# MoseleyBioinformaticsLab/pdb_eda

Measured on NVIDIA B200. Metric: voxels/s (atom-sphere voxels + blob-CCL voxels per pass of the voxel hot path), higher is better.
Workload: dtype f64

## Files before the change

include/pdbeda_b200.h:

```cpp
#ifndef PDBEDA_B200_H
#define PDBEDA_B200_H

#include <stdint.h>

#ifdef __cplusplus
extern "C" {
#endif

#define PE_ABI_VERSION 1

typedef enum pe_status {
    PE_OK = 0,
    PE_ERR_ARG = -1,
    PE_ERR_CUDA = -2,
    PE_ERR_CAPACITY = -3,
    PE_ERR_NO_DEVICE = -4
} pe_status;

typedef struct pe_geom {
    int32_t ncrs[3];
    int32_t crs_start[3];
    int32_t xyz_interval[3];
    int32_t crs_interval[3];
    int32_t unique_ncrs[3];
    int32_t map2xyz[3];
    int32_t map2crs[3];
    int32_t orthogonal;
    int32_t mv_perm[3];
    int32_t mv_fma;
    double grid_length[3];
    double origin[3];
    double ortho[9];
    double deortho[9];
} pe_geom;

int pe_abi_version(void);
const char *pe_last_error(void);
int pe_device_info(int32_t *sm_count, int32_t *cc_major, int32_t *cc_minor);

long long pe_launch_count(void);
void pe_profile_enable(int on);
void pe_profile_reset(void);
int pe_profile_entries(void);
int pe_profile_get(int index, const char **name, long long *count, double *total_ms);

int64_t pe_stats_workspace_bytes(void);
int pe_map_mean_std(const float *d_rho, int64_t n, double *d_out, void *d_ws, void *stream);
int pe_map_sum_abs(const float *d_rho, int64_t n, float cutoff, double *d_out, void *d_ws, void *stream);
int pe_sum_abs_f64(const double *d_values, int64_t n, float cutoff, double *d_out, void *d_ws, void *stream);

int pe_point_density(const pe_geom *g, const float *d_rho, int64_t n, const int32_t *d_crs, float *d_rho_out,
                     uint8_t *d_valid, void *stream);
int pe_xyz2crs(const pe_geom *g, int64_t n, const double *d_xyz, int32_t *d_crs, void *stream);
int pe_crs2xyz(const pe_geom *g, int64_t n, const int32_t *d_crs, double *d_xyz, void *stream);

#define PE_SPHERE_NOUT 8
int64_t pe_sphere_workspace_bytes(int64_t n_atoms);
int pe_sphere_union_warp_cycles(unsigned long long *out5);
int pe_sphere_sums(const pe_geom *g, const float *d_rho, int32_t n_atoms, const double *d_xyz,
                   const float *d_radius, int32_t n_groups, const int32_t *d_group_start, float cut_pos,
                   float cut_neg, double *d_out, void *d_ws, void *stream);
int pe_sphere_sums_atoms_and_groups(const pe_geom *g, const float *d_rho, int32_t n_atoms, const double *d_xyz,
                                    const float *d_atom_radius, float max_atom_radius, const float *d_group_radius,
                                    int32_t n_groups, const int32_t *d_group_start, float cut_pos, float cut_neg,
                                    double *d_out_atoms, double *d_out_groups, void *d_ws, void *stream);

typedef struct pe_sums_map {
    pe_geom geom;
    const float *d_rho;
    float cut_pos;
    float cut_neg;
} pe_sums_map;
int64_t pe_batch_sphere_sums_workspace_bytes(int64_t n_atoms);
int pe_batch_sphere_sums(int32_t n_maps, const pe_sums_map *d_maps, int32_t n_atoms, const double *d_xyz, const float *d_radius,
                         int32_t n_groups, const int32_t *d_group_map, const int32_t *d_group_start, const int32_t *d_atom_start,
                         double *d_out, void *d_ws, void *stream);

int pe_sphere_count(const pe_geom *g, const float *d_rho, int32_t n_atoms, const double *d_xyz,
                    const float *d_radius, float cutoff, int32_t *d_count, int32_t *d_box, void *stream);
int pe_sphere_fill(const pe_geom *g, const float *d_rho, int32_t n_atoms, const double *d_xyz,
                   const float *d_radius, float cutoff, const int64_t *d_offset, int32_t max_box_voxels,
                   int32_t *d_index, float *d_value, int32_t *d_label, void *stream);

int64_t pe_blob_workspace_bytes(const pe_geom *g, int64_t cap_voxels);
int pe_blob_stage_times(unsigned long long *out12);
int pe_blob_label(const pe_geom *g, const float *d_rho, float cut_pos, float cut_neg, int64_t cap_voxels,
                  int64_t cap_blobs, int64_t *d_counts, uint32_t *d_key, float *d_value, int32_t *d_label,
                  double *d_stats, void *d_ws, void *stream);

int64_t pe_slab_exchange_bytes(int64_t cap_blobs, int64_t cap_plane);
int64_t pe_slab_workspace_bytes(int32_t world, int64_t cap_blobs, int32_t u0, int32_t u1);
int pe_slab_boundary(const pe_geom *g_slab, int32_t u2_whole, int32_t s0, int32_t last_is_cut, const int64_t *d_counts,
                     int64_t cap_voxels, const uint32_t *d_key, const int32_t *d_label, int64_t cap_blobs, int64_t cap_plane,
                     void *d_exchange, void *d_ws, void *stream);
int pe_slab_merge(int32_t world, int32_t rank, const void *d_gathered, int64_t cap_blobs, int64_t cap_plane, int32_t u0,
                  int32_t u1, int32_t *d_new_number, int64_t *d_n_merged, void *d_ws, void *stream);
int pe_slab_relabel(const pe_geom *g_whole, int32_t u2_slab, int32_t s0, const int64_t *d_counts, int64_t cap_voxels,
                    const uint32_t *d_key, const float *d_value, int32_t *d_label, int64_t cap_blobs,
                    const int32_t *d_new_number, const int64_t *d_n_merged, int64_t cap_merged, double *d_stats, void *d_ws,
                    void *stream);
int pe_slab_status(const void *d_ws, void *stream, int32_t *bad);

int64_t pe_cluster_workspace_bytes(int64_t n);
int pe_cluster_crs(int64_t n, const int32_t *d_crs, int32_t *d_label, int64_t *d_nclusters, void *d_ws,
                   void *stream);
int pe_cluster_crs_grouped(int64_t n, const int32_t *d_crs, const int32_t *d_group, int32_t *d_label,
                           uint8_t *d_first, int64_t *d_nclusters, void *d_ws, void *stream);

int pe_crs_stats(const pe_geom *g, const float *d_rho, int64_t n, const int32_t *d_crs, const int32_t *d_label,
                 const uint8_t *d_take, int64_t n_clusters, double *d_stats, void *stream);

int pe_pair_metrics(const pe_geom *g, const float *d_rho_fo, const float *d_rho_diff, int64_t n, const int32_t *d_crs,
                    const int32_t *d_label, const uint8_t *d_take, int64_t n_groups, double *d_out, void *stream);

typedef struct pe_pair_map {
    pe_geom geom;
    const float *d_fo;
    const float *d_diff;
} pe_pair_map;
int64_t pe_pair_union_workspace_bytes(int32_t n_atoms);
int pe_pair_union_metrics(int32_t n_maps, const pe_pair_map *d_maps, int32_t n_groups, const int32_t *d_group_map,
                          const int32_t *d_group_start, const double *d_xyz, const float *d_radius, double *d_out, void *d_ws,
                          void *stream);

int64_t pe_overlap_workspace_bytes(int64_t n, int64_t cap_pairs);
int pe_overlap_pairs(int64_t n, const int32_t *d_crs, const int32_t *d_owner, const int32_t *d_group,
                     int64_t cap_pairs, int64_t *d_npairs, int32_t *d_pairs, void *d_ws, void *stream);

typedef struct pe_batch_map {
    pe_geom geom;
    const float *d_rho;
    float cutoff;
    int32_t atom_begin, atom_end;
    int32_t reserved;
} pe_batch_map;
int64_t pe_cloud_workspace_bytes(int64_t n_atoms, int64_t n_entries, int64_t n_residues, int64_t n_maps);
int pe_cloud_count(int32_t n_maps, const pe_batch_map *d_maps, int32_t n_atoms, const int32_t *d_atom_map, const double *d_xyz,
                   const float *d_radius, uint32_t *d_offset, int64_t *d_totals, void *d_scan_ws, uint32_t *d_box_bits, void *stream);
int pe_cloud_aggregate(int32_t n_maps, const pe_batch_map *d_maps, int32_t n_atoms, const int32_t *d_atom_map,
                       const double *d_xyz, const float *d_radius, const int32_t *d_atom_residue,
                       const int32_t *d_atom_local, const uint64_t *d_atom_bonded, const double *d_atom_electrons,
                       int32_t n_residues, const uint32_t *d_offset, int64_t n_entries, int32_t max_box_voxels,
                       double min_cloud_electrons, const uint32_t *d_box_bits, double *d_atom_out, double *d_map_out, void *d_ws,
                       void *stream);
int pe_cloud_status(const void *d_ws, void *stream, int32_t *bad);
int pe_cloud_statistics(int32_t n_maps, const pe_batch_map *d_maps, int32_t n_atoms, const double *d_atom_out,
                        const double *d_map_out, const double *d_atom_static, const int32_t *d_perm, int32_t n_segments,
                        const int32_t *d_seg_map, const int32_t *d_seg_type, const int32_t *d_seg_begin,
                        const int32_t *d_seg_end, int32_t max_segment, const double *d_unit_volume,
                        const double *d_current_slopes, double min_total_electrons, double *d_scratch, double *d_seg_out,
                        double *d_map_stats, void *stream);

int64_t pe_symmetry_workspace_bytes(int32_t n_atoms, int32_t n_ops);
int pe_symmetry_expand(const pe_geom *g, int32_t n_atoms, const double *d_xyz, int32_t n_ops, const double *d_rot,
                       const double *d_shift, const double *lo, const double *hi, int64_t cap, int64_t *d_count,
                       int32_t *d_atom, int32_t *d_image, double *d_out_xyz, void *d_ws, void *stream);

int pe_nearest_atom(int64_t n_blobs, const double *d_centroid, int64_t n_atoms, const double *d_coords,
                    int32_t *d_idx, double *d_dist, void *stream);

#ifdef __cplusplus
}
#endif
#endif
```

pdb_eda_b200/_lib.py:

```python
import ctypes
import os

_HERE = os.path.dirname(os.path.abspath(__file__))
LIB_PATH = os.path.join(_HERE, "csrc", "libpdbeda_b200.so")

PE_SPHERE_NOUT = 8


class PeGeom(ctypes.Structure):
    _fields_ = [
        ("ncrs", ctypes.c_int32 * 3),
        ("crs_start", ctypes.c_int32 * 3),
        ("xyz_interval", ctypes.c_int32 * 3),
        ("crs_interval", ctypes.c_int32 * 3),
        ("unique_ncrs", ctypes.c_int32 * 3),
        ("map2xyz", ctypes.c_int32 * 3),
        ("map2crs", ctypes.c_int32 * 3),
        ("orthogonal", ctypes.c_int32),
        ("mv_perm", ctypes.c_int32 * 3),
        ("mv_fma", ctypes.c_int32),
        ("grid_length", ctypes.c_double * 3),
        ("origin", ctypes.c_double * 3),
        ("ortho", ctypes.c_double * 9),
        ("deortho", ctypes.c_double * 9),
    ]


class PeBatchMap(ctypes.Structure):
    _fields_ = [("geom", PeGeom), ("d_rho", ctypes.c_void_p), ("cutoff", ctypes.c_float), ("atom_begin", ctypes.c_int32),
                ("atom_end", ctypes.c_int32), ("reserved", ctypes.c_int32)]


class PeSumsMap(ctypes.Structure):
    _fields_ = [("geom", PeGeom), ("d_rho", ctypes.c_void_p), ("cut_pos", ctypes.c_float), ("cut_neg", ctypes.c_float)]


class PePairMap(ctypes.Structure):
    _fields_ = [("geom", PeGeom), ("d_fo", ctypes.c_void_p), ("d_diff", ctypes.c_void_p)]


class PdbEdaLibError(RuntimeError):
    pass


_P = ctypes.c_void_p
_I32 = ctypes.c_int32
_I64 = ctypes.c_int64
_F32 = ctypes.c_float
_GEOM = ctypes.POINTER(PeGeom)

SIGNATURES = {
    "pe_abi_version": (ctypes.c_int, []),
    "pe_last_error": (ctypes.c_char_p, []),
    "pe_device_info": (ctypes.c_int, [ctypes.POINTER(_I32)] * 3),
    "pe_launch_count": (ctypes.c_longlong, []),
    "pe_profile_enable": (None, [ctypes.c_int]),
    "pe_profile_reset": (None, []),
    "pe_profile_entries": (ctypes.c_int, []),
    "pe_profile_get": (ctypes.c_int, [ctypes.c_int, ctypes.POINTER(ctypes.c_char_p), ctypes.POINTER(ctypes.c_longlong),
                                      ctypes.POINTER(ctypes.c_double)]),
    "pe_stats_workspace_bytes": (_I64, []),
    "pe_map_mean_std": (ctypes.c_int, [_P, _I64, _P, _P, _P]),
    "pe_map_sum_abs": (ctypes.c_int, [_P, _I64, _F32, _P, _P, _P]),
    "pe_sum_abs_f64": (ctypes.c_int, [_P, _I64, _F32, _P, _P, _P]),
    "pe_point_density": (ctypes.c_int, [_GEOM, _P, _I64, _P, _P, _P, _P]),
    "pe_xyz2crs": (ctypes.c_int, [_GEOM, _I64, _P, _P, _P]),
    "pe_crs2xyz": (ctypes.c_int, [_GEOM, _I64, _P, _P, _P]),
    "pe_sphere_workspace_bytes": (_I64, [_I64]),
    "pe_sphere_union_warp_cycles": (ctypes.c_int, [ctypes.POINTER(ctypes.c_ulonglong)]),
    "pe_sphere_sums": (ctypes.c_int, [_GEOM, _P, _I32, _P, _P, _I32, _P, _F32, _F32, _P, _P, _P]),
    "pe_sphere_sums_atoms_and_groups": (ctypes.c_int, [_GEOM, _P, _I32, _P, _P, _F32, _P, _I32, _P, _F32, _F32, _P, _P, _P, _P]),
    "pe_sphere_count": (ctypes.c_int, [_GEOM, _P, _I32, _P, _P, _F32, _P, _P, _P]),
    "pe_sphere_fill": (ctypes.c_int, [_GEOM, _P, _I32, _P, _P, _F32, _P, _I32, _P, _P, _P, _P]),
    "pe_blob_workspace_bytes": (_I64, [_GEOM, _I64]),
    "pe_blob_stage_times": (ctypes.c_int, [ctypes.POINTER(ctypes.c_ulonglong)]),
    "pe_blob_label": (ctypes.c_int, [_GEOM, _P, _F32, _F32, _I64, _I64, _P, _P, _P, _P, _P, _P, _P]),
    "pe_cluster_workspace_bytes": (_I64, [_I64]),
    "pe_cluster_crs": (ctypes.c_int, [_I64, _P, _P, _P, _P, _P]),
    "pe_cluster_crs_grouped": (ctypes.c_int, [_I64, _P, _P, _P, _P, _P, _P, _P]),
    "pe_crs_stats": (ctypes.c_int, [_GEOM, _P, _I64, _P, _P, _P, _I64, _P, _P]),
    "pe_pair_metrics": (ctypes.c_int, [_GEOM, _P, _P, _I64, _P, _P, _P, _I64, _P, _P]),
    "pe_batch_sphere_sums_workspace_bytes": (_I64, [_I64]),
    "pe_batch_sphere_sums": (ctypes.c_int, [_I32, _P, _I32, _P, _P, _I32, _P, _P, _P, _P, _P, _P]),
    "pe_pair_union_workspace_bytes": (_I64, [_I32]),
    "pe_pair_union_metrics": (ctypes.c_int, [_I32, _P, _I32, _P, _P, _P, _P, _P, _P, _P]),
    "pe_overlap_workspace_bytes": (_I64, [_I64, _I64]),
    "pe_overlap_pairs": (ctypes.c_int, [_I64, _P, _P, _P, _I64, _P, _P, _P, _P]),
    "pe_symmetry_workspace_bytes": (_I64, [_I32, _I32]),
    "pe_symmetry_expand": (ctypes.c_int, [_GEOM, _I32, _P, _I32, _P, _P, ctypes.POINTER(ctypes.c_double),
                                          ctypes.POINTER(ctypes.c_double), _I64, _P, _P, _P, _P, _P, _P]),
    "pe_nearest_atom": (ctypes.c_int, [_I64, _P, _I64, _P, _P, _P, _P]),
    "pe_slab_exchange_bytes": (_I64, [_I64, _I64]),
    "pe_slab_workspace_bytes": (_I64, [_I32, _I64, _I32, _I32]),
    "pe_slab_boundary": (ctypes.c_int, [_GEOM, _I32, _I32, _I32, _P, _I64, _P, _P, _I64, _I64, _P, _P, _P]),
    "pe_slab_merge": (ctypes.c_int, [_I32, _I32, _P, _I64, _I64, _I32, _I32, _P, _P, _P, _P]),
    "pe_slab_relabel": (ctypes.c_int, [_GEOM, _I32, _I32, _P, _I64, _P, _P, _P, _I64, _P, _P, _I64, _P, _P, _P]),
    "pe_slab_status": (ctypes.c_int, [_P, _P, ctypes.POINTER(_I32)]),
    "pe_cloud_workspace_bytes": (_I64, [_I64, _I64, _I64, _I64]),
    "pe_cloud_count": (ctypes.c_int, [_I32, _P, _I32, _P, _P, _P, _P, _P, _P, _P, _P]),
    "pe_cloud_aggregate": (ctypes.c_int, [_I32, _P, _I32, _P, _P, _P, _P, _P, _P, _P, _I32, _P, _I64, _I32, ctypes.c_double, _P, _P, _P,
                                          _P, _P]),
    "pe_cloud_status": (ctypes.c_int, [_P, _P, ctypes.POINTER(_I32)]),
    "pe_cloud_statistics": (ctypes.c_int, [_I32, _P, _I32, _P, _P, _P, _P, _I32, _P, _P, _P, _P, _I32, _P, _P, ctypes.c_double, _P, _P,
                                           _P, _P]),
}

_lib = None


def load():
    global _lib
    if _lib is not None:
        return _lib
    if not os.path.isfile(LIB_PATH):
        raise PdbEdaLibError(
            "%s not found: build it with `python -c 'import __graft_entry__ as g; g.build()'` or "
            "`make -C pdb_eda_b200/csrc` (there is no CPU fallback)" % LIB_PATH)
    lib = ctypes.CDLL(LIB_PATH)
    for name, (restype, argtypes) in SIGNATURES.items():
        fn = getattr(lib, name)
        fn.restype = restype
        fn.argtypes = argtypes
    if lib.pe_abi_version() != 1:
        raise PdbEdaLibError("libpdbeda_b200.so ABI version %d, expected 1" % lib.pe_abi_version())
    _lib = lib
    return lib


def check(rc, what):
    if rc != 0:
        msg = load().pe_last_error()
        raise PdbEdaLibError("%s failed (%d): %s" % (what, rc, msg.decode("utf-8", "replace") if msg else "?"))


def require_device():
    lib = load()
    sm, major, minor = _I32(0), _I32(0), _I32(0)
    check(lib.pe_device_info(ctypes.byref(sm), ctypes.byref(major), ctypes.byref(minor)), "pe_device_info")
    return sm.value, major.value, minor.value


def profile(enable=None, reset=False):
    lib = load()
    if reset:
        lib.pe_profile_reset()
    if enable is not None:
        lib.pe_profile_enable(1 if enable else 0)
        return None
    out = {}
    for i in range(lib.pe_profile_entries()):
        name, count, ms = ctypes.c_char_p(), ctypes.c_longlong(0), ctypes.c_double(0.0)
        if lib.pe_profile_get(i, ctypes.byref(name), ctypes.byref(count), ctypes.byref(ms)) == 0:
            out[name.value.decode()] = (count.value, ms.value)
    return out


def launch_count():
    return load().pe_launch_count()
```

pdb_eda_b200/csrc/pe_blob.cu:

```cuda
#include <cooperative_groups.h>
#include "pe_common.cuh"

namespace cg = cooperative_groups;

namespace pe {

constexpr int kBmpTx = 32;
constexpr int kBmpTy = 8;
constexpr int kSparseThreads = 512;
constexpr int kSegShift = 9;
constexpr int kSegWords = 1 << kSegShift;
constexpr int kChunkShift = 9;
constexpr int kChunkSmem = 4096;
constexpr int kScanBlocksPerSm = 2;
constexpr int kQueueCap = 160;
constexpr int kPoolWords = (kSparseThreads / 32) * 3 * kQueueCap > kChunkSmem ? (kSparseThreads / 32) * 3 * kQueueCap : kChunkSmem;
static_assert((1 << kChunkShift) == kSparseThreads, "a ranking chunk is one block of voxels");

struct BlobPlan {
    int U0, U1, U2, W;
    int64_t nwords;
    int64_t nwords_pad;
    int64_t nseg;
    int64_t cap;
// ... 88 lines not shown
                }
            }
        } else {
            for (int j = 0; j < nbits; ++j) {
#pragma unroll
                for (int i = 0; i < VEC; ++i) {
                    const float e = (i == 0 || c + i < NC) ? __ldg(p + (int64_t)j * plane + i) : 0.f;
                    pos[i] |= (e >= cpos) ? (1u << j) : 0u;
                    neg[i] |= (e <= cneg) ? (1u << j) : 0u;
                }
            }
        }
#pragma unroll
        for (int i = 0; i < VEC; ++i) {
            accp[i][q] = use_pos ? pos[i] : 0u;
            accn[i][q] = use_neg ? neg[i] : 0u;
        }
    }
#pragma unroll
    for (int i = 0; i < VEC; ++i) {
        if (c + i < U0) {
            const int64_t widx = ((int64_t)(c + i) * U1 + r) * W + w_begin;
            *reinterpret_cast<uint4 *>(bmp_pos + widx) = make_uint4(accp[i][0], accp[i][1], accp[i][2], accp[i][3]);
            *reinterpret_cast<uint4 *>(bmp_neg + widx) = make_uint4(accn[i][0], accn[i][1], accn[i][2], accn[i][3]);
            const int np = __popc(accp[i][0]) + __popc(accp[i][1]) + __popc(accp[i][2]) + __popc(accp[i][3]);
            const int nn = __popc(accn[i][0]) + __popc(accn[i][1]) + __popc(accn[i][2]) + __popc(accn[i][3]);
            if (np) atomicAdd(segcount + (widx >> kSegShift), (uint32_t)np);
            if (nn) atomicAdd(segcount + ((nwords_pad + widx) >> kSegShift), (uint32_t)nn);
        }
    }
}

__device__ unsigned long long g_stage_ns[12];
__device__ __forceinline__ void stamp(int i) {
    if (blockIdx.x == 0 && threadIdx.x == 0) {
        unsigned long long t;
        asm volatile("mov.u64 %0, %%globaltimer;" : "=l"(t));
        g_stage_ns[i] = t;
    }
}

struct SparseArgs {
    const float *rho;
    int NC, NR, U1, U2, W;
    int64_t nwords_pad, cap, cap_blobs;
    int nseg;
    int p1_blocks;
    int p1_per_sm;
    int *sm_rank;
    const uint32_t *bmp;
    const uint32_t *segcount;
    uint32_t *base;
    uint32_t *parent;
    uint2 *flags;
    uint32_t *coarse;
    int64_t nchunk_cap;
    int64_t *counts;
    uint32_t *key;
    float *value;
    int32_t *label;
    double *stats;
};

__device__ __forceinline__ uint32_t block_sum_u32(uint32_t v, uint32_t *smem ) {
    const int lane = threadIdx.x & 31, w = threadIdx.x >> 5;
    v = (uint32_t)warp_sum((int)v);
    __syncthreads();
    if (lane == 0) smem[w] = v;
    __syncthreads();
    uint32_t t = 0;
    for (int i = 0; i < (int)(blockDim.x >> 5); ++i) t += smem[i];
    return t;
}

__device__ __forceinline__ uint32_t uf_union_root(uint32_t *parent, uint32_t a, uint32_t b) {
    for (;;) {
        a = uf_find_halve(parent, a);
        b = uf_find_halve(parent, b);
        if (a == b) return a;
        if (a < b) {
            const uint32_t t = a;
            a = b;
            b = t;
        }
        const uint32_t old = atomicMin(parent + a, b);
        if (old == a) return b;
        a = old;
    }
}

__device__ __forceinline__ uint32_t roots_below(const uint2 *__restrict__ flags, const uint32_t *cpre, uint32_t x) {
    const uint2 f = __ldcg(flags + (x >> 5));
    return cpre[x >> kChunkShift] + f.y + (uint32_t)__popc(f.x & ((1u << (x & 31u)) - 1u));
}

__global__ void __launch_bounds__(kSparseThreads, 3) blob_sparse_kernel(const __grid_constant__ pe_geom g, const SparseArgs a) {
    cg::grid_group grid = cg::this_grid();
    __shared__ uint32_t smem[32];
    __shared__ uint32_t pool[kPoolWords];
    uint32_t *cpre_s = pool;
    const int lane = threadIdx.x & 31, warp = threadIdx.x >> 5;
    const int nb = gridDim.x, b = blockIdx.x;
    const int warps_per_block = kSparseThreads >> 5;
    stamp(0);

    uint32_t n0 = 0, n_all = 0;
    __shared__ int scan_index;
    if (threadIdx.x == 0) {
        unsigned smid;
        asm volatile("mov.u32 %0, %%smid;" : "=r"(smid));
        int idx = -1;
        if (a.p1_blocks >= nb) idx = b;
        else if (atomicAdd(a.sm_rank + (smid < 254u ? smid : 254u), 1) < a.p1_per_sm) idx = atomicAdd(a.sm_rank + 255, 1);
        scan_index = idx;
    }
    __syncthreads();
    const int bi = scan_index;
    if (bi >= 0 && bi < a.p1_blocks) {
        const int nwarps = a.p1_blocks * warps_per_block;
        const int spw = (a.nseg + nwarps - 1) / nwarps;
        const int seg_class1 = (int)(a.nwords_pad >> kSegShift);
        const int sb = min(bi * warps_per_block * spw, a.nseg);
        {
            const int seg_begin = min(sb + warp * spw, a.nseg), seg_end = min(seg_begin + spw, a.nseg);
            for (int64_t i = ((int64_t)seg_begin << kSegShift) + 32 * lane; i < ((int64_t)seg_end << kSegShift); i += 32 * 32)
                asm volatile("prefetch.global.L2 [%0];" ::"l"(a.bmp + i));
        }
        uint32_t before;
        {
            uint32_t s_before = 0, s0 = 0, s_all = 0;
            constexpr int kBatch = 8;
            for (int i0 = threadIdx.x; i0 < a.nseg; i0 += kSparseThreads * kBatch) {
                uint32_t v[kBatch];
#pragma unroll
                for (int j = 0; j < kBatch; ++j) {
                    const int i = i0 + j * kSparseThreads;
                    v[j] = i < a.nseg ? __ldg(a.segcount + i) : 0u;
                }
#pragma unroll
                for (int j = 0; j < kBatch; ++j) {
                    const int i = i0 + j * kSparseThreads;
                    s_all += v[j];
                    if (i < sb) s_before += v[j];
                    if (i < seg_class1) s0 += v[j];
                }
            }
            before = block_sum_u32(s_before, smem);
            n0 = block_sum_u32(s0, smem);
            n_all = block_sum_u32(s_all, smem);
        }
        const bool overflow = (int64_t)n0 > a.cap || (int64_t)(n_all - n0) > a.cap;
        if (bi == 0 && threadIdx.x == 0) {
            a.counts[0] = (int64_t)n0;
            a.counts[2] = (int64_t)(n_all - n0);
            if (overflow) a.counts[4] = 1;
        }
        if (!overflow) {
            const int seg_begin = min(sb + warp * spw, a.nseg), seg_end = min(seg_begin + spw, a.nseg);
            uint32_t mine = 0;
            for (int i = sb + lane; i < seg_begin; i += 32) mine += a.segcount[i];
            uint32_t run = before + (uint32_t)warp_sum((int)mine);
            uint32_t carry = 0u;
            if (seg_begin < seg_end && seg_begin > 0) carry = a.bmp[((int64_t)seg_begin << kSegShift) - 1];
            const int64_t w_end = (int64_t)seg_end << kSegShift;
            uint32_t *queue = pool + warp * (3 * kQueueCap);
            int qn = 0;
            uint4 next = make_uint4(0u, 0u, 0u, 0u);
            if (seg_begin < seg_end) next = __ldcg(reinterpret_cast<const uint4 *>(a.bmp + ((int64_t)seg_begin << kSegShift) + 4 * lane));
            for (int64_t i0 = (int64_t)seg_begin << kSegShift; i0 < w_end; i0 += 128) {
                const int64_t widx0 = i0 + 4 * lane;
                const uint4 wv = next;
                if (i0 + 128 < w_end) next = __ldcg(reinterpret_cast<const uint4 *>(a.bmp + widx0 + 128));
                const int c4 = __popc(wv.x) + __popc(wv.y) + __popc(wv.z) + __popc(wv.w);
                const int excl = warp_excl_scan(c4, lane);
                uint32_t p = run + (uint32_t)excl;
                run += (uint32_t)__shfl_sync(kFull, excl + c4, 31);
                uint32_t prevw = __shfl_up_sync(kFull, wv.w, 1);
                if (lane == 0) prevw = carry;
                carry = __shfl_sync(kFull, wv.w, 31);
                const uint32_t words[4] = {wv.x, wv.y, wv.z, wv.w};
#pragma unroll
                for (int q = 0; q < 4; ++q) {
                    const uint32_t word = words[q];
                    const unsigned act = __ballot_sync(kFull, word != 0u);
                    if (word) {
                        const int slot = qn + __popc(act & ((1u << lane) - 1u));
                        const uint32_t pw = q == 0 ? prevw : words[q > 0 ? q - 1 : 0];
                        queue[slot] = (uint32_t)(widx0 + q);
                        queue[kQueueCap + slot] = p | (pw & 0x80000000u);
                        queue[2 * kQueueCap + slot] = word;
                        p += (uint32_t)__popc(word);
                    }
                    qn += __popc(act);
                }
                const bool last = i0 + 128 >= w_end;
                if (qn <= kQueueCap - 128 && !last) continue;
                __syncwarp();
                for (int e = lane; e < qn; e += 32) {
                    const uint32_t widx = queue[e], pp = queue[kQueueCap + e], word = queue[2 * kQueueCap + e];
                    const uint32_t p_first = pp & 0x7fffffffu;
                    const int k = (int64_t)widx >= a.nwords_pad ? 1 : 0;
                    const uint32_t local = widx - (k ? (uint32_t)a.nwords_pad : 0u);
                    const uint32_t colrow = local / (uint32_t)a.W;
                    const int w = (int)(local - colrow * (uint32_t)a.W);
                    const int64_t out0 = (int64_t)k * a.cap - (k ? (int64_t)n0 : 0);
                    const bool prev_last = (w > 0) && (pp >> 31);
                    a.base[widx] = p_first;
                    const uint32_t starts = word & ~((word << 1) | (prev_last ? 1u : 0u));
                    const uint32_t keybase = colrow * (uint32_t)a.U2 + (uint32_t)w * 32u;
                    uint32_t rest = word, pv = p_first;
                    while (rest) {
                        const int bit = __ffs(rest) - 1;
                        rest &= rest - 1;
                        const uint32_t below = starts & ((2u << bit) - 1u);
                        uint32_t par;
                        if (below) {
                            const int sbit = 31 - __clz(below);
                            par = p_first + (uint32_t)__popc(word & ((1u << sbit) - 1u));
                        } else {
                            par = p_first - 1;
                        }
                        a.key[out0 + pv] = keybase + (uint32_t)bit;
                        a.parent[pv] = par;
                        ++pv;
                    }
                }
                qn = 0;
                __syncwarp();
            }
        }
    }
    grid.sync();
    stamp(1);
    if (!(bi >= 0 && bi < a.p1_blocks)) {
        n0 = (uint32_t)__ldcg(a.counts + 0);
        n_all = n0 + (uint32_t)__ldcg(a.counts + 2);
    }
    if (a.p1_blocks < nb && __ldcg(a.sm_rank + 255) != a.p1_blocks) {
        if (b == 0 && threadIdx.x == 0) a.counts[4] = 2;
        return;
    }
    if (__ldcg(a.counts + 4) != 0) return;
    const int64_t n = (int64_t)n_all;
    const uint32_t n1 = n_all - n0;

    const int64_t gstride = (int64_t)nb * kSparseThreads;
    const int64_t gtid = (int64_t)b * kSparseThreads + threadIdx.x;
    {
        const int64_t rows0 = min((int64_t)n0, a.cap_blobs) * 8, rows1 = min((int64_t)n1, a.cap_blobs) * 8;
        for (int64_t i = gtid; i < rows0; i += gstride) a.stats[i] = 0.0;
        for (int64_t i = gtid; i < rows1; i += gstride) a.stats[a.cap_blobs * 8 + i] = 0.0;
    }
    for (int64_t i = gtid; i < n; i += gstride) {
        const int k = i >= (int64_t)n0 ? 1 : 0;
        const int64_t oi = (int64_t)k * a.cap + (i - (k ? (int64_t)n0 : 0));
        const uint32_t kk = __ldcg(a.key + oi);
        const int s = (int)(kk % (uint32_t)a.U2);
        const uint32_t colrow = kk / (uint32_t)a.U2;
        const int r = (int)(colrow % (uint32_t)a.U1), c = (int)(colrow / (uint32_t)a.U1);
        const int w = s >> 5, bit = s & 31;
        const uint32_t *bmp = a.bmp + (k ? a.nwords_pad : 0);
        const uint32_t *base = a.base + (k ? a.nwords_pad : 0);
        const float dens = __ldg(a.rho + ((int64_t)s * a.NR + r) * a.NC + c);
        int64_t nw[4];
        bool ok[4];
        ok[0] = c > 0 && r > 0;
        ok[1] = c > 0;
        ok[2] = c > 0 && r + 1 < a.U1;
        ok[3] = r > 0;
        nw[0] = ((int64_t)(c - 1) * a.U1 + r - 1) * a.W + w;
        nw[1] = nw[0] + a.W;
        nw[2] = nw[1] + a.W;
        nw[3] = ((int64_t)c * a.U1 + r - 1) * a.W + w;
        uint32_t B[4], Bm[4], Bp[4];
#pragma unroll
        for (int j = 0; j < 4; ++j) {
            B[j] = ok[j] ? __ldcg(bmp + nw[j]) : 0u;
            Bm[j] = (ok[j] && bit == 0 && w > 0) ? __ldcg(bmp + nw[j] - 1) : 0u;
            Bp[j] = (ok[j] && bit == 31 && w + 1 < a.W) ? __ldcg(bmp + nw[j] + 1) : 0u;
        }
        uint32_t sel[4];
#pragma unroll
        for (int j = 0; j < 4; ++j) {
            uint32_t m = 0;
            if ((B[j] >> bit) & 1u) {
                m = 1u;
            } else {
                if (bit > 0 && ((B[j] >> (bit - 1)) & 1u)) m |= 2u;
                if (bit < 31 && ((B[j] >> (bit + 1)) & 1u)) m |= 4u;
                if (Bm[j] >> 31) m |= 8u;
                if (Bp[j] & 1u) m |= 16u;
            }
            sel[j] = m;
        }
        if (sel[1] & 1u) {
            sel[0] = sel[2] = sel[3] = 0u;
        } else if (sel[3] & 1u) {
            sel[0] = sel[1] = 0u;
        } else if (sel[0] & 1u) {
            sel[1] = sel[3] = 0u;
        } else if (sel[2] & 1u) {
            sel[1] = 0u;
        } else {
#pragma unroll
            for (int side = 0; side < 2; ++side) {
                const uint32_t bits = side ? (4u | 16u) : (2u | 8u);
                if (sel[1] & bits) {
                    sel[0] &= ~bits;
// ... 43 lines not shown
        }
        const uint32_t fw = __ballot_sync(kFull, isroot);
        if (lane == 0) wcnt[warp] = (uint32_t)__popc(fw);
        __syncthreads();
        uint32_t fine = 0, tot = 0;
        for (int j = 0; j < warps_per_block; ++j) {
            const uint32_t v = wcnt[j];
            if (j < warp) fine += v;
            tot += v;
        }
        if (lane == 0) a.flags[(chunk << (kChunkShift - 5)) + warp] = make_uint2(fw, fine);
        if (threadIdx.x == 0) a.coarse[chunk] = tot;
        __syncthreads();
    }
    grid.sync();
    stamp(3);

    const uint32_t *cpre = cpre_s;
    uint32_t n_roots;
    if (nchunks <= kChunkSmem) {
        constexpr int kPer = kChunkSmem / kSparseThreads;
        uint32_t v[kPer], sum = 0;
#pragma unroll
        for (int j = 0; j < kPer; ++j) {
            const int64_t ci = (int64_t)threadIdx.x * kPer + j;
            v[j] = ci < nchunks ? __ldcg(a.coarse + ci) : 0u;
            sum += v[j];
        }
        const uint32_t wex = (uint32_t)warp_excl_scan((int)sum, lane);
        __syncthreads();
        if (lane == 31) wcnt[warp] = wex + sum;
        __syncthreads();
        uint32_t off = wex;
        uint32_t all = 0;
        for (int j = 0; j < warps_per_block; ++j) {
            const uint32_t t = wcnt[j];
            if (j < warp) off += t;
            all += t;
        }
#pragma unroll
        for (int j = 0; j < kPer; ++j) {
            cpre_s[threadIdx.x * kPer + j] = off;
            off += v[j];
        }
        n_roots = all;
        __syncthreads();
    } else {
        uint32_t *gpre = a.coarse + a.nchunk_cap;
        if (b == 0) {
            __shared__ uint32_t carry_s;
            if (threadIdx.x == 0) carry_s = 0u;
            __syncthreads();
            for (int64_t c0 = 0; c0 < nchunks; c0 += kSparseThreads) {
                const int64_t ci = c0 + threadIdx.x;
                const uint32_t v = ci < nchunks ? __ldcg(a.coarse + ci) : 0u;
                const uint32_t wex = (uint32_t)warp_excl_scan((int)v, lane);
                if (lane == 31) wcnt[warp] = wex + v;
                __syncthreads();
                uint32_t off = carry_s + wex, all = 0;
                for (int j = 0; j < warps_per_block; ++j) {
                    const uint32_t t = wcnt[j];
                    if (j < warp) off += t;
                    all += t;
                }
                if (ci < nchunks) gpre[ci] = off;
                __syncthreads();
                if (threadIdx.x == 0) carry_s += all;
                __syncthreads();
            }
            if (threadIdx.x == 0) gpre[nchunks] = carry_s;
        }
        grid.sync();
        cpre = gpre;
        n_roots = __ldcg(gpre + nchunks);
    }
    const uint32_t nb0 = n0 == n_all ? n_roots : roots_below(a.flags, cpre, n0);
    const uint32_t nb1 = n_roots - nb0;
    if (b == 0 && threadIdx.x == 0) {
        a.counts[1] = (int64_t)nb0;
        a.counts[3] = (int64_t)nb1;
    }
    if ((int64_t)nb0 > a.cap_blobs || (int64_t)nb1 > a.cap_blobs) {
        if (b == 0 && threadIdx.x == 0) a.counts[4] = 1;
        return;
    }
    for (int64_t i0 = gtid - lane; i0 < n; i0 += gstride) {
        const int64_t i = i0 + lane;
        const bool live = i < n;
        int32_t blob = -1;
        double v[8] = {0, 0, 0, 0, 0, 0, 0, 0};
        if (live) {
            const int k = i >= (int64_t)n0 ? 1 : 0;
            const int64_t oi = (int64_t)k * a.cap + (i - (k ? (int64_t)n0 : 0));
            const uint32_t gr = roots_below(a.flags, cpre, __ldcg(a.parent + i));
            blob = (int32_t)(gr - (k ? nb0 : 0u));
            a.label[oi] = blob;
            blob += k ? (int32_t)a.cap_blobs : 0;
            const uint32_t kk = __ldcg(a.key + oi);
            const int s = (int)(kk % (uint32_t)a.U2);
            const uint32_t colrow = kk / (uint32_t)a.U2;
            const int r = (int)(colrow % (uint32_t)a.U1), c = (int)(colrow / (uint32_t)a.U1);
            double x, y, z;
            crs2xyz(g, c, r, s, x, y, z);
            const double d = (double)__ldcg(a.value + oi);
            v[0] = 1.0;
            v[1] = d;
            v[2] = __dmul_rn(d, x);
            v[3] = __dmul_rn(d, y);
            v[4] = __dmul_rn(d, z);
            v[5] = x;
            v[6] = y;
            v[7] = z;
        }
        const int32_t prev = __shfl_up_sync(kFull, blob, 1);
        const bool head = (lane == 0) || (prev != blob);
        const unsigned heads = __ballot_sync(kFull, head);
        const int segno = __popc(heads & (0xffffffffu >> (31 - lane)));
#pragma unroll
        for (int o = 1; o < 32; o <<= 1) {
            const int seg_o = __shfl_down_sync(kFull, segno, o);
            const bool take = (lane + o < 32) && (seg_o == segno);
#pragma unroll
            for (int q = 0; q < 8; ++q) {
                const double other = __shfl_down_sync(kFull, v[q], o);
                if (take) v[q] += other;
            }
        }
        if (live && head) {
            double *st = a.stats + (int64_t)blob * 8;
#pragma unroll
            for (int q = 0; q < 8; ++q) atomicAdd(st + q, v[q]);
        }
    }
    stamp(4);
}

}

using namespace pe;

extern "C" {

int pe_blob_stage_times(unsigned long long *out12) {
    PE_CHECK_ARG(out12 != nullptr, "pe_blob_stage_times: null pointer");
    PE_CUDA(cudaMemcpyFromSymbol(out12, g_stage_ns, sizeof(unsigned long long) * 12));
    return PE_OK;
}

int64_t pe_blob_workspace_bytes(const pe_geom *g, int64_t cap_voxels) {
    if (!g || cap_voxels < 0) return -1;
    return make_plan(g, cap_voxels).total;
}

int pe_blob_label(const pe_geom *g, const float *d_rho, float cut_pos, float cut_neg, int64_t cap_voxels,
                  int64_t cap_blobs, int64_t *d_counts, uint32_t *d_key, float *d_value, int32_t *d_label,
                  double *d_stats, void *d_ws, void *stream) {
    if (int rc = check_geom(g)) return rc;
    PE_CHECK_ARG(d_rho && d_counts && d_key && d_value && d_label && d_stats && d_ws, "pe_blob_label: null pointer");
    PE_CHECK_ARG(cap_voxels > 0 && cap_blobs > 0, "pe_blob_label: capacities must be positive");
    PE_CHECK_ARG(cap_voxels < (1ll << 30), "pe_blob_label: cap_voxels must be below 2^30");
    PE_CHECK_ARG(!(cut_pos < 0.f) && !(cut_neg > 0.f), "pe_blob_label: cut_pos must be >= 0 and cut_neg <= 0");
    PE_CHECK_ARG(cut_pos == cut_pos && cut_neg == cut_neg, "pe_blob_label: NaN cutoff");
    const BlobPlan p = make_plan(g, cap_voxels);
    PE_CHECK_ARG((int64_t)p.U0 * p.U1 * p.U2 < (1ll << 32), "pe_blob_label: unique volume too large for 32-bit keys");
    PE_CHECK_ARG(p.nwords_pad < (1ll << 31), "pe_blob_label: bit planes too large");
    cudaStream_t st = (cudaStream_t)stream;
    char *ws = (char *)d_ws;
    const int NC = g->ncrs[0], NR = g->ncrs[1];
    uint32_t *bmp = (uint32_t *)(ws + p.off_bmp);
    const bool use_pos = cut_pos > 0.f, use_neg = cut_neg < 0.f;

    PE_CUDA(cudaMemsetAsync(d_counts, 0, 5 * sizeof(int64_t), st));
    uint32_t *segcount = (uint32_t *)(ws + p.off_seg);
    PE_CUDA(cudaMemsetAsync(segcount, 0, (size_t)align_up(p.nseg * 4, 256) + 1024, st));
    {
        const bool vec4 = (NC % 4 == 0) && (((uintptr_t)d_rho & 15u) == 0);
        const int vec = vec4 ? 4 : 1;
        const int tx = kBmpTx, ty = kBmpTy;
        dim3 block(tx, ty, 1);
        dim3 grid(p.W / kWordsPerThread, (p.U0 + tx * vec - 1) / (tx * vec), (p.U1 + ty - 1) / ty);
        PE_CHECK_ARG(grid.y <= 65535 && grid.z <= 65535, "pe_blob_label: map too large for the launch grid");
        if (vec4)
            PE_LAUNCH("threshold_bitmap_kernel", st, threshold_bitmap_kernel<4><<<grid, block, 0, st>>>(
                d_rho, NC, NR, p.U0, p.U1, p.U2, p.W, cut_pos, cut_neg, use_pos, use_neg, bmp, bmp + p.nwords_pad, p.nwords_pad, segcount));
        else
            PE_LAUNCH("threshold_bitmap_kernel", st, threshold_bitmap_kernel<1><<<grid, block, 0, st>>>(
                d_rho, NC, NR, p.U0, p.U1, p.U2, p.W, cut_pos, cut_neg, use_pos, use_neg, bmp, bmp + p.nwords_pad, p.nwords_pad, segcount));
        PE_LAUNCH_CHECK();
    }
    SparseArgs a;
    a.rho = d_rho;
    a.NC = NC;
    a.NR = NR;
    a.U1 = p.U1;
    a.U2 = p.U2;
    a.W = p.W;
    a.nwords_pad = p.nwords_pad;
    a.cap = p.cap;
    a.cap_blobs = cap_blobs;
    a.nseg = (int)p.nseg;
    a.bmp = bmp;
    a.segcount = segcount;
    a.base = (uint32_t *)(ws + p.off_base);
    a.parent = (uint32_t *)(ws + p.off_parent);
    a.flags = (uint2 *)(ws + p.off_flags);
    a.coarse = (uint32_t *)(ws + p.off_coarse);
    a.nchunk_cap = p.nchunk_cap;
    a.counts = d_counts;
    a.key = d_key;
    a.value = d_value;
    a.label = d_label;
    a.stats = d_stats;
    static int blocks_per_sm = 0;
    if (blocks_per_sm == 0) {
        PE_CUDA(cudaOccupancyMaxActiveBlocksPerMultiprocessor(&blocks_per_sm, blob_sparse_kernel, kSparseThreads, 0));
        PE_CHECK_ARG(blocks_per_sm > 0, "pe_blob_label: the sparse kernel does not fit an SM");
    }
    const int nblocks = sm_count() * (blocks_per_sm < 3 ? blocks_per_sm : 3);
    a.p1_per_sm = blocks_per_sm == 3 ? kScanBlocksPerSm : (blocks_per_sm < 3 ? blocks_per_sm : 3);
    a.p1_blocks = sm_count() * a.p1_per_sm;
    a.sm_rank = (int *)(ws + p.off_seg + align_up(p.nseg * 4, 256));
    pe_geom geom = *g;
    void *args[] = {(void *)&geom, (void *)&a};
    PE_LAUNCH("blob_sparse_kernel", st,
              PE_CUDA(cudaLaunchCooperativeKernel((const void *)blob_sparse_kernel, dim3(nblocks), dim3(kSparseThreads), args, 0, st)));
    PE_LAUNCH_CHECK();
    return PE_OK;
}

}
```

pdb_eda_b200/pipeline.py:

```python
import ctypes

import numpy as np
import torch

from . import _device
from ._device import _ptr, _stream
from ._lib import PE_SPHERE_NOUT, check


class VoxelPass:
    def __init__(self, densityDev, diffDev, xyz, radii, residueStart, regionRadius=3.5, densityCutoff=None,
                 diffCutoff=None, capVoxels=None, capBlobs=None):
        self.dens = densityDev
        self.diff = diffDev
        dev = densityDev.device
        self.device = dev
        self.lib = densityDev.lib
        self.xyz = _device._as_dev(xyz, torch.float64, dev, (-1, 3))
        self.n_atoms = self.xyz.shape[0]
        self.radii = _device._as_dev(radii, torch.float32, dev, (-1,))
        self.max_radius = float(self.radii.max().item()) if self.n_atoms else 0.0
        self.region_radii = torch.full((self.n_atoms,), float(np.float32(regionRadius)), dtype=torch.float32, device=dev)
        self.res_start = _device._as_dev(residueStart, torch.int32, dev, (-1,))
        self.n_res = self.res_start.numel() - 1
        if densityCutoff is None:
            m, s = densityDev.mean_std()
            densityCutoff = m + 1.5 * s
        if diffCutoff is None:
            m, s = diffDev.mean_std()
            diffCutoff = m + 3.0 * s
        self.density_cut = float(np.float32(densityCutoff))
        self.diff_cut = float(np.float32(diffCutoff))
        self.cloud_out = torch.empty((self.n_atoms, PE_SPHERE_NOUT), dtype=torch.float64, device=dev)
        self.region_out = torch.empty((self.n_res, PE_SPHERE_NOUT), dtype=torch.float64, device=dev)
        self.sphere_ws = torch.empty(max(int(self.lib.pe_sphere_workspace_bytes(self.n_atoms)), 256), dtype=torch.uint8, device=dev)
        g = diffDev.geom
        nvox = g.unique_ncrs[0] * g.unique_ncrs[1] * g.unique_ncrs[2]
        self.n_blob_voxels = nvox
        self.cap_voxels = int(capVoxels or max(4096, nvox // 64))
        self.cap_blobs = int(capBlobs or max(1024, self.cap_voxels // 4))
        self.blob_counts = torch.zeros(5, dtype=torch.int64, device=dev)
        self.blob_key = torch.empty(2 * self.cap_voxels, dtype=torch.int32, device=dev)
        self.blob_value = torch.empty(2 * self.cap_voxels, dtype=torch.float32, device=dev)
        self.blob_label = torch.empty(2 * self.cap_voxels, dtype=torch.int32, device=dev)
        self.blob_stats = torch.empty((2 * self.cap_blobs, 8), dtype=torch.float64, device=dev)
        self.blob_ws = torch.empty(max(int(self.lib.pe_blob_workspace_bytes(ctypes.byref(g), self.cap_voxels)), 256),
                                   dtype=torch.uint8, device=dev)

    def spheres(self):
        check(self.lib.pe_sphere_sums_atoms_and_groups(
            ctypes.byref(self.dens.geom), _ptr(self.dens.rho), self.n_atoms, _ptr(self.xyz), _ptr(self.radii),
            ctypes.c_float(self.max_radius), _ptr(self.region_radii), self.n_res, _ptr(self.res_start),
            ctypes.c_float(self.density_cut), ctypes.c_float(0.0), _ptr(self.cloud_out), _ptr(self.region_out),
            _ptr(self.sphere_ws), _stream()), "pe_sphere_sums_atoms_and_groups")

    def blobs(self):
        check(self.lib.pe_blob_label(ctypes.byref(self.diff.geom), _ptr(self.diff.rho), ctypes.c_float(self.diff_cut),
                                     ctypes.c_float(-self.diff_cut), self.cap_voxels, self.cap_blobs, _ptr(self.blob_counts),
                                     _ptr(self.blob_key), _ptr(self.blob_value), _ptr(self.blob_label), _ptr(self.blob_stats),
                                     _ptr(self.blob_ws), _stream()), "pe_blob_label")

    def step(self):
        if getattr(self, "_side", None) is None:
            self._side = torch.cuda.Stream(device=self.device)
            self._fork, self._join = torch.cuda.Event(), torch.cuda.Event()
        main = torch.cuda.current_stream()
        self._fork.record(main)
        self._side.wait_event(self._fork)
        with torch.cuda.stream(self._side):
            self.blobs()
        self.spheres()
        self._join.record(self._side)
        main.wait_event(self._join)

    def stepFromHost(self, hostDensity, hostDiff, hostXyz=None):
        if getattr(self, "_copy", None) is None:
            self._copy = torch.cuda.Stream(device=self.device)
            self._ev = [torch.cuda.Event() for _ in range(3)]
        ev_free, ev_dens, ev_diff = self._ev
        main = torch.cuda.current_stream()
        ev_free.record(main)
        self._copy.wait_event(ev_free)
        with torch.cuda.stream(self._copy):
            self.dens.rho.copy_(hostDensity.view(-1), non_blocking=True)
            if hostXyz is not None:
                self.xyz.copy_(hostXyz, non_blocking=True)
            ev_dens.record(self._copy)
            self.diff.rho.copy_(hostDiff.view(-1), non_blocking=True)
            ev_diff.record(self._copy)
        main.wait_event(ev_dens)
        self.spheres()
        main.wait_event(ev_diff)
        self.blobs()
        return self.results()

    def _host_buffers(self):
        if getattr(self, "_h", None) is None:
            pin = lambda t: torch.empty(t.shape, dtype=t.dtype).pin_memory()
            self._h = {"cloud": pin(self.cloud_out), "region": pin(self.region_out), "counts": pin(self.blob_counts),
                       "key": pin(self.blob_key), "label": pin(self.blob_label), "stats": pin(self.blob_stats)}
        return self._h

    def results(self):
        h = self._host_buffers()
        h["cloud"].copy_(self.cloud_out, non_blocking=True)
        h["region"].copy_(self.region_out, non_blocking=True)
        h["counts"].copy_(self.blob_counts, non_blocking=True)
        torch.cuda.current_stream().synchronize()
        counts = h["counts"].numpy().copy()
        if counts[4]:
            raise RuntimeError("blob capacities too small: %s voxels / %s blobs needed" % (max(counts[0], counts[2]), max(counts[1], counts[3])))
        spans = []
        for k in range(2):
            nfg, nb = int(counts[2 * k]), int(counts[2 * k + 1])
            v0, b0 = k * self.cap_voxels, k * self.cap_blobs
            h["key"][v0:v0 + nfg].copy_(self.blob_key[v0:v0 + nfg], non_blocking=True)
            h["label"][v0:v0 + nfg].copy_(self.blob_label[v0:v0 + nfg], non_blocking=True)
            h["stats"][b0:b0 + nb].copy_(self.blob_stats[b0:b0 + nb], non_blocking=True)
            spans.append((v0, nfg, b0, nb))
        torch.cuda.current_stream().synchronize()
        out = {"cloud": h["cloud"].numpy(), "region": h["region"].numpy(), "blob_counts": counts}
        for (v0, nfg, b0, nb), tag in zip(spans, ("green", "red")):
            out[tag] = {"key": h["key"].numpy()[v0:v0 + nfg], "label": h["label"].numpy()[v0:v0 + nfg], "stats": h["stats"].numpy()[b0:b0 + nb]}
        return out

    def unit_counts(self):
        cloud = float(self.cloud_out[:, 0].sum().item())
        region = float(self.region_out[:, 0].sum().item())
        return cloud, region, float(self.n_blob_voxels)
```

Baseline: 483.9 billion.

## Split blob labeling so only thresholding overlaps spheres, sparse CCL runs after

Blob labeling is split into a threshold-bitmap entry point and a sparse-labeling entry point. In step(), only the bitmap pass runs on the side stream alongside the sphere kernels, and the sparse kernel, which sizes its grid to fill every SM, runs on the main stream after the join so it no longer competes with the sphere kernels for SMs. The counts memset is dropped and the sparse kernel writes the count fields itself. The cost is that the sparse stage is now serialized after the spheres instead of overlapping with them.

After: 488.1 billion (median of 6 runs). Within noise of the previous version (+0.9%).

```diff
diff --git a/include/pdbeda_b200.h b/include/pdbeda_b200.h
--- a/include/pdbeda_b200.h
+++ b/include/pdbeda_b200.h
@@ -87,6 +87,12 @@
 int pe_blob_label(const pe_geom *g, const float *d_rho, float cut_pos, float cut_neg, int64_t cap_voxels,
                   int64_t cap_blobs, int64_t *d_counts, uint32_t *d_key, float *d_value, int32_t *d_label,
                   double *d_stats, void *d_ws, void *stream);
+int pe_blob_label_threshold(const pe_geom *g, const float *d_rho, float cut_pos, float cut_neg, int64_t cap_voxels,
+                            int64_t cap_blobs, int64_t *d_counts, uint32_t *d_key, float *d_value, int32_t *d_label,
+                            double *d_stats, void *d_ws, void *stream);
+int pe_blob_label_sparse(const pe_geom *g, const float *d_rho, float cut_pos, float cut_neg, int64_t cap_voxels,
+                         int64_t cap_blobs, int64_t *d_counts, uint32_t *d_key, float *d_value, int32_t *d_label,
+                         double *d_stats, void *d_ws, void *stream);
 
 int64_t pe_slab_exchange_bytes(int64_t cap_blobs, int64_t cap_plane);
 int64_t pe_slab_workspace_bytes(int32_t world, int64_t cap_blobs, int32_t u0, int32_t u1);
diff --git a/pdb_eda_b200/_lib.py b/pdb_eda_b200/_lib.py
--- a/pdb_eda_b200/_lib.py
+++ b/pdb_eda_b200/_lib.py
@@ -75,6 +75,8 @@
     "pe_blob_workspace_bytes": (_I64, [_GEOM, _I64]),
     "pe_blob_stage_times": (ctypes.c_int, [ctypes.POINTER(ctypes.c_ulonglong)]),
     "pe_blob_label": (ctypes.c_int, [_GEOM, _P, _F32, _F32, _I64, _I64, _P, _P, _P, _P, _P, _P, _P]),
+    "pe_blob_label_threshold": (ctypes.c_int, [_GEOM, _P, _F32, _F32, _I64, _I64, _P, _P, _P, _P, _P, _P, _P]),
+    "pe_blob_label_sparse": (ctypes.c_int, [_GEOM, _P, _F32, _F32, _I64, _I64, _P, _P, _P, _P, _P, _P, _P]),
     "pe_cluster_workspace_bytes": (_I64, [_I64]),
     "pe_cluster_crs": (ctypes.c_int, [_I64, _P, _P, _P, _P, _P]),
     "pe_cluster_crs_grouped": (ctypes.c_int, [_I64, _P, _P, _P, _P, _P, _P, _P]),
diff --git a/pdb_eda_b200/csrc/pe_blob.cu b/pdb_eda_b200/csrc/pe_blob.cu
--- a/pdb_eda_b200/csrc/pe_blob.cu
+++ b/pdb_eda_b200/csrc/pe_blob.cu
@@ -264,8 +264,10 @@
         const bool overflow = (int64_t)n0 > a.cap || (int64_t)(n_all - n0) > a.cap;
         if (bi == 0 && threadIdx.x == 0) {
             a.counts[0] = (int64_t)n0;
+            a.counts[1] = 0;
             a.counts[2] = (int64_t)(n_all - n0);
-            if (overflow) a.counts[4] = 1;
+            a.counts[3] = 0;
+            a.counts[4] = overflow ? 1 : 0;
         }
         if (!overflow) {
             const int seg_begin = min(sb + warp * spw, a.nseg), seg_end = min(seg_begin + spw, a.nseg);
@@ -615,34 +617,39 @@
     return make_plan(g, cap_voxels).total;
 }
 
-int pe_blob_label(const pe_geom *g, const float *d_rho, float cut_pos, float cut_neg, int64_t cap_voxels,
-                  int64_t cap_blobs, int64_t *d_counts, uint32_t *d_key, float *d_value, int32_t *d_label,
-                  double *d_stats, void *d_ws, void *stream) {
+}
+
+namespace {
+
+enum BlobPart { kBlobThreshold = 1, kBlobSparse = 2 };
+
+int blob_label_parts(int parts, const char *fn, const pe_geom *g, const float *d_rho, float cut_pos, float cut_neg,
+                     int64_t cap_voxels, int64_t cap_blobs, int64_t *d_counts, uint32_t *d_key, float *d_value, int32_t *d_label,
+                     double *d_stats, void *d_ws, void *stream) {
     if (int rc = check_geom(g)) return rc;
-    PE_CHECK_ARG(d_rho && d_counts && d_key && d_value && d_label && d_stats && d_ws, "pe_blob_label: null pointer");
-    PE_CHECK_ARG(cap_voxels > 0 && cap_blobs > 0, "pe_blob_label: capacities must be positive");
-    PE_CHECK_ARG(cap_voxels < (1ll << 30), "pe_blob_label: cap_voxels must be below 2^30");
-    PE_CHECK_ARG(!(cut_pos < 0.f) && !(cut_neg > 0.f), "pe_blob_label: cut_pos must be >= 0 and cut_neg <= 0");
-    PE_CHECK_ARG(cut_pos == cut_pos && cut_neg == cut_neg, "pe_blob_label: NaN cutoff");
+    PE_CHECK_ARG(d_rho && d_counts && d_key && d_value && d_label && d_stats && d_ws, "%s: null pointer", fn);
+    PE_CHECK_ARG(cap_voxels > 0 && cap_blobs > 0, "%s: capacities must be positive", fn);
+    PE_CHECK_ARG(cap_voxels < (1ll << 30), "%s: cap_voxels must be below 2^30", fn);
+    PE_CHECK_ARG(!(cut_pos < 0.f) && !(cut_neg > 0.f), "%s: cut_pos must be >= 0 and cut_neg <= 0", fn);
+    PE_CHECK_ARG(cut_pos == cut_pos && cut_neg == cut_neg, "%s: NaN cutoff", fn);
     const BlobPlan p = make_plan(g, cap_voxels);
-    PE_CHECK_ARG((int64_t)p.U0 * p.U1 * p.U2 < (1ll << 32), "pe_blob_label: unique volume too large for 32-bit keys");
-    PE_CHECK_ARG(p.nwords_pad < (1ll << 31), "pe_blob_label: bit planes too large");
+    PE_CHECK_ARG((int64_t)p.U0 * p.U1 * p.U2 < (1ll << 32), "%s: unique volume too large for 32-bit keys", fn);
+    PE_CHECK_ARG(p.nwords_pad < (1ll << 31), "%s: bit planes too large", fn);
     cudaStream_t st = (cudaStream_t)stream;
     char *ws = (char *)d_ws;
     const int NC = g->ncrs[0], NR = g->ncrs[1];
     uint32_t *bmp = (uint32_t *)(ws + p.off_bmp);
     const bool use_pos = cut_pos > 0.f, use_neg = cut_neg < 0.f;
-
-    PE_CUDA(cudaMemsetAsync(d_counts, 0, 5 * sizeof(int64_t), st));
     uint32_t *segcount = (uint32_t *)(ws + p.off_seg);
-    PE_CUDA(cudaMemsetAsync(segcount, 0, (size_t)align_up(p.nseg * 4, 256) + 1024, st));
-    {
+
+    if (parts & kBlobThreshold) {
         const bool vec4 = (NC % 4 == 0) && (((uintptr_t)d_rho & 15u) == 0);
         const int vec = vec4 ? 4 : 1;
         const int tx = kBmpTx, ty = kBmpTy;
         dim3 block(tx, ty, 1);
         dim3 grid(p.W / kWordsPerThread, (p.U0 + tx * vec - 1) / (tx * vec), (p.U1 + ty - 1) / ty);
-        PE_CHECK_ARG(grid.y <= 65535 && grid.z <= 65535, "pe_blob_label: map too large for the launch grid");
+        PE_CHECK_ARG(grid.y <= 65535 && grid.z <= 65535, "%s: map too large for the launch grid", fn);
+        PE_CUDA(cudaMemsetAsync(segcount, 0, (size_t)align_up(p.nseg * 4, 256) + 1024, st));
         if (vec4)
             PE_LAUNCH("threshold_bitmap_kernel", st, threshold_bitmap_kernel<4><<<grid, block, 0, st>>>(
                 d_rho, NC, NR, p.U0, p.U1, p.U2, p.W, cut_pos, cut_neg, use_pos, use_neg, bmp, bmp + p.nwords_pad, p.nwords_pad, segcount));
@@ -651,6 +658,7 @@
                 d_rho, NC, NR, p.U0, p.U1, p.U2, p.W, cut_pos, cut_neg, use_pos, use_neg, bmp, bmp + p.nwords_pad, p.nwords_pad, segcount));
         PE_LAUNCH_CHECK();
     }
+    if (!(parts & kBlobSparse)) return PE_OK;
     SparseArgs a;
     a.rho = d_rho;
     a.NC = NC;
@@ -677,7 +685,7 @@
     static int blocks_per_sm = 0;
     if (blocks_per_sm == 0) {
         PE_CUDA(cudaOccupancyMaxActiveBlocksPerMultiprocessor(&blocks_per_sm, blob_sparse_kernel, kSparseThreads, 0));
-        PE_CHECK_ARG(blocks_per_sm > 0, "pe_blob_label: the sparse kernel does not fit an SM");
+        PE_CHECK_ARG(blocks_per_sm > 0, "%s: the sparse kernel does not fit an SM", fn);
     }
     const int nblocks = sm_count() * (blocks_per_sm < 3 ? blocks_per_sm : 3);
     a.p1_per_sm = blocks_per_sm == 3 ? kScanBlocksPerSm : (blocks_per_sm < 3 ? blocks_per_sm : 3);
@@ -692,3 +700,28 @@
 }
 
 }
+
+extern "C" {
+
+int pe_blob_label(const pe_geom *g, const float *d_rho, float cut_pos, float cut_neg, int64_t cap_voxels,
+                  int64_t cap_blobs, int64_t *d_counts, uint32_t *d_key, float *d_value, int32_t *d_label,
+                  double *d_stats, void *d_ws, void *stream) {
+    return blob_label_parts(kBlobThreshold | kBlobSparse, "pe_blob_label", g, d_rho, cut_pos, cut_neg, cap_voxels, cap_blobs,
+                            d_counts, d_key, d_value, d_label, d_stats, d_ws, stream);
+}
+
+int pe_blob_label_threshold(const pe_geom *g, const float *d_rho, float cut_pos, float cut_neg, int64_t cap_voxels,
+                            int64_t cap_blobs, int64_t *d_counts, uint32_t *d_key, float *d_value, int32_t *d_label,
+                            double *d_stats, void *d_ws, void *stream) {
+    return blob_label_parts(kBlobThreshold, "pe_blob_label_threshold", g, d_rho, cut_pos, cut_neg, cap_voxels, cap_blobs,
+                            d_counts, d_key, d_value, d_label, d_stats, d_ws, stream);
+}
+
+int pe_blob_label_sparse(const pe_geom *g, const float *d_rho, float cut_pos, float cut_neg, int64_t cap_voxels,
+                         int64_t cap_blobs, int64_t *d_counts, uint32_t *d_key, float *d_value, int32_t *d_label,
+                         double *d_stats, void *d_ws, void *stream) {
+    return blob_label_parts(kBlobSparse, "pe_blob_label_sparse", g, d_rho, cut_pos, cut_neg, cap_voxels, cap_blobs,
+                            d_counts, d_key, d_value, d_label, d_stats, d_ws, stream);
+}
+
+}
diff --git a/pdb_eda_b200/pipeline.py b/pdb_eda_b200/pipeline.py
--- a/pdb_eda_b200/pipeline.py
+++ b/pdb_eda_b200/pipeline.py
@@ -54,11 +54,12 @@
             ctypes.c_float(self.density_cut), ctypes.c_float(0.0), _ptr(self.cloud_out), _ptr(self.region_out),
             _ptr(self.sphere_ws), _stream()), "pe_sphere_sums_atoms_and_groups")
 
-    def blobs(self):
-        check(self.lib.pe_blob_label(ctypes.byref(self.diff.geom), _ptr(self.diff.rho), ctypes.c_float(self.diff_cut),
-                                     ctypes.c_float(-self.diff_cut), self.cap_voxels, self.cap_blobs, _ptr(self.blob_counts),
-                                     _ptr(self.blob_key), _ptr(self.blob_value), _ptr(self.blob_label), _ptr(self.blob_stats),
-                                     _ptr(self.blob_ws), _stream()), "pe_blob_label")
+    def blobs(self, part=""):
+        name = "pe_blob_label_" + part if part else "pe_blob_label"
+        check(getattr(self.lib, name)(ctypes.byref(self.diff.geom), _ptr(self.diff.rho), ctypes.c_float(self.diff_cut),
+                                      ctypes.c_float(-self.diff_cut), self.cap_voxels, self.cap_blobs, _ptr(self.blob_counts),
+                                      _ptr(self.blob_key), _ptr(self.blob_value), _ptr(self.blob_label), _ptr(self.blob_stats),
+                                      _ptr(self.blob_ws), _stream()), name)
 
     def step(self):
         if getattr(self, "_side", None) is None:
@@ -68,10 +69,11 @@
         self._fork.record(main)
         self._side.wait_event(self._fork)
         with torch.cuda.stream(self._side):
-            self.blobs()
+            self.blobs("threshold")
+            self._join.record(self._side)
         self.spheres()
-        self._join.record(self._side)
         main.wait_event(self._join)
+        self.blobs("sparse")
 
     def stepFromHost(self, hostDensity, hostDiff, hostXyz=None):
         if getattr(self, "_copy", None) is None:
diff --git a/profiles/c2_beside.py b/profiles/c2_beside.py
--- /dev/null
+++ b/profiles/c2_beside.py
@@ -0,0 +1,87 @@
+#!/usr/bin/env python3
+import argparse
+import ctypes
+import os
+import subprocess
+import sys
+
+import numpy as np
+import torch
+
+ROOT = os.path.dirname(os.path.dirname(os.path.abspath(__file__)))
+sys.path.insert(0, ROOT)
+from pdb_eda_b200 import _device, _lib, ccp4, synthetic
+
+if os.environ.get("PE_LIB"):
+    _lib.LIB_PATH = os.path.abspath(os.environ["PE_LIB"])
+from pdb_eda_b200.pipeline import VoxelPass
+import bench
+
+
+def timed(fn, reps):
+    for _ in range(3):
+        fn()
+    torch.cuda.synchronize()
+    e0, e1 = torch.cuda.Event(enable_timing=True), torch.cuda.Event(enable_timing=True)
+    e0.record()
+    for _ in range(reps):
+        fn()
+    e1.record()
+    torch.cuda.synchronize()
+    return e0.elapsed_time(e1) * 1e3 / reps
+
+
+def main():
+    ap = argparse.ArgumentParser()
+    ap.add_argument("--tag", default="tree")
+    ap.add_argument("--reps", type=int, default=200)
+    ap.add_argument("--trace")
+    args = ap.parse_args()
+    print(subprocess.run(["nvidia-smi", "--query-gpu=name,power.limit,clocks.max.sm", "--format=csv"], capture_output=True,
+                         text=True).stdout.strip())
+    work = bench.build_workload(bench.FULL, seed=2)
+    n, cell = work["n"], work["cell"]
+    geom = _device.geom_from_header(ccp4.DensityHeader.fromFileHeader(synthetic.ccp4Header((n, n, n), cell, (n, n, n))))
+    dens = _device.DeviceMap(geom, torch.from_numpy(work["fofc2"].reshape(-1)).cuda())
+    diff = _device.DeviceMap(geom, torch.from_numpy(work["fofc"].reshape(-1)).cuda())
+    vp = VoxelPass(dens, diff, work["xyz"].astype(np.float64), work["radii"], work["res_start"], bench.REGION_RADIUS)
+    lib = _lib.load()
+    beside = hasattr(lib, "pe_blob_label_beside")
+    print("[%s] spheres alone          %8.2f us" % (args.tag, timed(vp.spheres, args.reps)))
+    print("[%s] pe_blob_label alone    %8.2f us" % (args.tag, timed(vp.blobs, args.reps)))
+    if beside:
+        print("[%s] pe_blob_label_beside alone %8.2f us" % (args.tag, timed(lambda: vp.blobs(beside=True), args.reps)))
+        d = (ctypes.c_ulonglong * 4)()
+        lib.pe_blob_beside_diag(d)
+        print("[%s] beside diag: blocks sharing an SM %d, P0 %.1f us, kernel %.1f us (last launch)"
+              % (args.tag, d[0], (d[2] - d[1]) / 1e3, (d[3] - d[1]) / 1e3))
+    print("[%s] step                   %8.2f us" % (args.tag, timed(vp.step, args.reps)))
+    if beside:
+        lib.pe_blob_beside_diag(d)
+        print("[%s] beside diag in the step: blocks sharing an SM %d, P0 %.1f us, kernel %.1f us (last launch)"
+              % (args.tag, d[0], (d[2] - d[1]) / 1e3, (d[3] - d[1]) / 1e3))
+    if args.trace:
+        from torch.profiler import ProfilerActivity, profile
+        for _ in range(5):
+            vp.step()
+        torch.cuda.synchronize()
+        with profile(activities=[ProfilerActivity.CUDA]) as prof:
+            for _ in range(3):
+                vp.step()
+            torch.cuda.synchronize()
+        ev = sorted((e for e in prof.events() if e.device_type.name == "CUDA"), key=lambda e: e.time_range.start)
+        os.makedirs(args.trace, exist_ok=True)
+        last = [e for e in ev if "sphere_union" in e.name][-1]
+        t0 = min(e.time_range.start for e in ev if e.time_range.end >= last.time_range.start - 20)
+        path = os.path.join(args.trace, args.tag + "_step.csv")
+        with open(path, "w") as f:
+            f.write("kernel,start_us,end_us,dur_us\n")
+            for e in ev:
+                if e.time_range.start >= t0:
+                    f.write("%s,%.1f,%.1f,%.1f\n" % (e.name.split("(")[0][:60], e.time_range.start - t0, e.time_range.end - t0,
+                                                      e.time_range.end - e.time_range.start))
+        print(open(path).read())
+
+
+if __name__ == "__main__":
+    main()
```
